# gylien/scale-letkf

Measured on AMD Instinct MI355X. Metric: grid-point LETKF solves/sec, higher is better.
Workload: dtype f64

## Files before the change

### __graft_entry__.py

```python
import importlib.util
import os
import subprocess
import sys

ROOT = os.path.dirname(os.path.abspath(__file__))
PKG_DIR = os.path.join(ROOT, "scale-letkf_amd")


def load_package():
    if "scale_letkf_amd" in sys.modules:
        return sys.modules["scale_letkf_amd"]
    spec = importlib.util.spec_from_file_location("scale_letkf_amd", os.path.join(PKG_DIR, "__init__.py"),
                                                  submodule_search_locations=[PKG_DIR])
    mod = importlib.util.module_from_spec(spec)
    sys.modules["scale_letkf_amd"] = mod
    spec.loader.exec_module(mod)
    return mod


def build():
    pkg = load_package()
    pkg.build()
    subprocess.check_call(["make", "-j4", "-C", PKG_DIR, "CHECKED=1"], stdout=2)
    subprocess.check_call(["make", "-C", os.path.join(ROOT, "oracle"), "oracle"])
    if os.path.isdir("/root/reference/common") and os.path.exists("/opt/rocm/bin/amdflang"):
        subprocess.check_call(["make", "-C", os.path.join(ROOT, "oracle"), "ref"])
    shim_mk = os.path.join(PKG_DIR, "fortran", "Makefile")
    if os.path.exists(shim_mk) and os.path.exists("/opt/rocm/bin/amdflang"):
        subprocess.check_call(["make", "-C", os.path.join(PKG_DIR, "fortran")])
    pkg.lib()


def smoke():
    import numpy as np
    import torch
    sys.path.insert(0, os.path.join(ROOT, "tests"))
    import _oracle
    from _cases import das_case, relerr
    pkg = load_package()
    assert torch.cuda.is_available(), "smoke() needs a GPU"
    dev = torch.device("cuda:0")
    c = das_case(k=20, nv=11, npts=16, nobs_tot=300, n_mean=40, seed=11)
    prm = _oracle.DasParams(k=20, nv=11, det_run=0, infl_adaptive=0, relax_to_inflated_prior=0, relax_alpha=0.0,
                            relax_alpha_spread=0.95, q_update_top=0.0, q_sprd_max=0.0, iv_p=4, iv_q_first=5,
                            iv_q_last=10, nthreads=1)
    ref = _oracle.das_points(prm, c["obs_off"], c["obs_idx"], c["rdiag"], c["rloc"], c["ensval"], c["dep"],
                             c["beta"], c["infl"], c["gues"], c["sp"], c["sm"], c["sv"])
    t = lambda a: torch.from_numpy(np.ascontiguousarray(a)).to(dev)
    ctx = pkg.Context(0, torch.cuda.current_stream().cuda_stream)
    anal = torch.zeros(c["gues"].size, dtype=torch.float64, device=dev)
    status = torch.full((c["npts"],), -1, dtype=torch.int32, device=dev)
    ctx.das_points(20, 11, t(c["obs_off"]), t(c["obs_idx"]), t(c["rdiag"]), t(c["rloc"]), t(c["ensval"]), c["kld"],
                   t(c["dep"]), t(c["infl"]), t(c["gues"]), anal, c["sp"], c["sm"], c["sv"], beta=t(c["beta"]),
                   relax_alpha_spread=0.95, status=status)
    torch.cuda.synchronize()
    assert int(status.abs().max()) == 0, status
    got = anal.cpu().numpy().reshape(11, c["nens"], c["npts"])[:, :20, :]
    exp = ref["anal"].reshape(11, c["nens"], c["npts"])[:, :20, :]
    err = relerr(got, exp)
    assert err < 1e-10, err
    print(f"smoke ok: 16 points, k=20, max rel err vs oracle {err:.2e}")


if __name__ == "__main__":
    build()
    print("build ok")
```

### scale-letkf_amd/csrc/letkf_jacobi_dev.h

```cpp
#pragma once
#include <hip/hip_runtime.h>

#include "letkf_lane_dev.h"

namespace letkf {
namespace jacobi_dev {

using namespace lane_dev;

typedef double v4d __attribute__((ext_vector_type(4)));

template <int NW>
__device__ __forceinline__ void psync() {
  if constexpr (NW == 1) wave_lds_sync();
  else __syncthreads();
}
template <int NW>
__device__ __forceinline__ bool pany(bool v) {
  if constexpr (NW == 1) return __builtin_amdgcn_ballot_w64(v) != 0ull;
  else return __syncthreads_or(v) != 0;
}

constexpr double kRotTol2W = 1e-30;
#ifndef LETKF_EARLY_TOL2
#define LETKF_EARLY_TOL2 1e-16
#endif
#ifndef LETKF_EARLY_T2
#define LETKF_EARLY_T2 1e-12
#endif
#ifndef LETKF_STOP_TOL2
#define LETKF_STOP_TOL2 1e-24
#endif
constexpr double kStopTol2W = LETKF_STOP_TOL2;
constexpr double kEarlyTol2W = LETKF_EARLY_TOL2;
constexpr double kEarlyT2W = LETKF_EARLY_T2;
constexpr double kEarlyTW = 1e-6;
static_assert(LETKF_EARLY_T2 == 1e-12, "kEarlyTW is its square root");

__device__ __forceinline__ double fast_rsqrt(double x) {
  const double y = __builtin_amdgcn_rsq(x);
  const double e = fma(-x * y, y, 1.0);
  const double q = e * fma(0.375, e, 0.5);
  return fma(y, q, y);
}
__device__ __forceinline__ double fast_rsqrt1(double x) { return __builtin_amdgcn_rsq(x); }
__device__ __forceinline__ double fast_rcp1(double x) { return __builtin_amdgcn_rcp(x); }
__device__ __forceinline__ double fast_rcp(double x) {
  double r = __builtin_amdgcn_rcp(x);
  double e = fma(-x, r, 1.0);
  r = fma(r, e, r);
  e = fma(-x, r, 1.0);
  return fma(r, e, r);
}

template <int CTRL>
__device__ __forceinline__ double dpp_shift_keep(double old, double v) {
  const int lo = __builtin_amdgcn_update_dpp(__double2loint(old), __double2loint(v), CTRL, 0xF, 0xF, false);
  const int hi = __builtin_amdgcn_update_dpp(__double2hiint(old), __double2hiint(v), CTRL, 0xF, 0xF, false);
  return __hiloint2double(hi, lo);
}
__device__ __forceinline__ double copy64(double v) {
  double t;
  asm("v_mov_b64 %0, %1" : "=v"(t) : "v"(v));
  return t;
}
__device__ __forceinline__ double slot_sum(double v) {
  const auto lo = __builtin_amdgcn_permlane32_swap(__double2loint(v), __double2loint(v), false, false);
  const auto hi = __builtin_amdgcn_permlane32_swap(__double2hiint(v), __double2hiint(v), false, false);
  return __hiloint2double(hi[0], lo[0]) + __hiloint2double(hi[1], lo[1]);
}

__device__ __forceinline__ double slot_sum_c64(double v) {
  const double t = copy64(v);
  const auto lo = __builtin_amdgcn_permlane32_swap(__double2loint(v), __double2loint(t), false, false);
  const auto hi = __builtin_amdgcn_permlane32_swap(__double2hiint(v), __double2hiint(t), false, false);
  return __hiloint2double(hi[0], lo[0]) + __hiloint2double(hi[1], lo[1]);
}

template <int NW>
__device__ __forceinline__ double slot_sum_nw(double v, double* xs, int& ph) {
  if constexpr (NW == 1) {
    return slot_sum_c64(v);
  } else {
    const int t = threadIdx.x & 127;
    xs[ph * 128 + t] = v;
    __syncthreads();
    const double o = xs[ph * 128 + (t ^ 64)];
    ph ^= 1;
    return v + o;
  }
}

template <int KR, int NW, int RC = 24, bool EARLY = true, bool INPLACE = false>
__device__ __forceinline__ int jacobi_split(double (&g)[KR], const int k, const int max_sweep, double* lds,
                                            int* pairs_out = nullptr, int* conv_out = nullptr, const double stop_tol2 = kStopTol2W) {
  static_assert(KR % 2 == 0, "row halves");
  constexpr int H = KR / 2;
  static_assert(RC % 2 == 0, "RC rows per conversion chunk: RC * 64 NW doubles of LDS");
  constexpr bool ENDS = NW == 1;
  static_assert(!ENDS || KR <= 64, "one wave: k <= 62, lane 31 stays switched off");
  constexpr int NL = 64 * NW;
  int lane = threadIdx.x & (NL - 1);
  if constexpr (NW == 2) asm volatile("" : "+v"(lane));
  const int slot = (NW == 1) ? (lane & 31) : (lane & 63), par = (NW == 1) ? (lane >> 5) : (lane >> 6);
  int ph = 0;
  const int ncol = (k + 1) & ~1;
  const int S = ncol >> 1;
  double xa[H], xb[H], xf[INPLACE ? 1 : H];
#pragma unroll
  for (int r0 = 0; r0 < KR; r0 += RC) {
    psync<NW>();
#pragma unroll
    for (int r = r0; r < r0 + RC && r < KR; ++r) lds[(r - r0) * NL + lane] = g[r];
    psync<NW>();
#pragma unroll
    for (int rr = r0 / 2; rr < (r0 + RC) / 2 && rr < H; ++rr) {
      const double2 v2 = *reinterpret_cast<const double2*>(&lds[(2 * rr + par - r0) * NL + 2 * slot]);
      xa[rr] = v2.x;
      xb[rr] = v2.y;
    }
  }
  int sweep = 0, pairs_done = 0, conv = 0;
  const bool act = slot < S;
  const bool rows = NW == 1 || act;
  if (NW == 2 || act) {
    const bool hasL = act && slot > 0, hasR = act && slot + 1 < S;
    const unsigned long long hasRm = __builtin_amdgcn_ballot_w64(hasR);
    double alA = 0.0, alB = 0.0, isA = 1.0, isB = 1.0, scA = 1.0, scB = 1.0;
    const double endR = hasR ? -0.0 : 1.0, endL = hasL ? -0.0 : 1.0;
    int quiet = 0, quiet2 = 0, pairs = 0, vph = 0;
    bool done = false;
    for (; sweep < max_sweep && !done; ++sweep) {
      double a0 = 0.0, b0 = 0.0;
      if (rows) {
#pragma unroll
        for (int rr = 0; rr < H; ++rr) {
          xa[rr] *= isA;
          xb[rr] *= isB;
          a0 = fma(xa[rr], xa[rr], a0);
          b0 = fma(xb[rr], xb[rr], b0);
        }
      }
      alA = slot_sum_nw<NW>(a0, lds, ph);
      alB = slot_sum_nw<NW>(b0, lds, ph);
      isA = isB = scA = scB = 1.0;
      for (int t = 0; t < ncol && !done; t += 2) {
        unsigned long long notconv = 0, notconv2 = 0;
        {
          double p0 = 0.0, p1 = 0.0;
          if (rows) {
#pragma unroll
            for (int rr = 0; rr < H; ++rr) {
              if (rr & 1) p1 = fma(xa[rr], xb[rr], p1);
              else p0 = fma(xa[rr], xb[rr], p0);
            }
          }
// ... 178 lines not shown
```

### scale-letkf_amd/csrc/letkf_trio.hip

```cpp
#include <hip/hip_runtime.h>
#include <stdint.h>

#include <type_traits>

#include "letkf_device.h"
#include "letkf_jacobi_dev.h"
#include "letkf_lane_dev.h"
#include "letkf_sched_dev.h"

namespace letkf {

namespace {

using namespace jacobi_dev;
using namespace lane_dev;

template <int KR, int P>
struct TrioLds {
  static constexpr int PSZ = (KR + 2) * KR;
  static constexpr int kSC = P > 3 ? 192 : 256;
  static constexpr int park = 0;
  static constexpr int lam = park + P * PSZ;
  static constexpr int st = lam + P * 32;
  static constexpr int work = st + P * 8;
// ... 42 lines not shown
    quiet[p] = quiet2[p] = pdone[p] = 0;
    sdone[p] = segm[p] == 0ull;
  }
  int pairs = 0;
  if (act) {
    const int colA = 2 * sin, colB = colA + 1;
    double xa[H], xb[H], xf[H];
#pragma unroll
    for (int rr = 0; rr < H; ++rr) {
      xa[rr] = base[colA * KR + 2 * rr + par];
      xb[rr] = base[colB * KR + 2 * rr + par];
    }
    const bool hasL = sin > 0, hasR = sin + 1 < S;
    const unsigned long long hasRm = __builtin_amdgcn_ballot_w64(hasR);
    double alA = 0.0, alB = 0.0, isA = 1.0, isB = 1.0, scA = 1.0, scB = 1.0;
    bool live = true;
    bool alldone = false;
    for (int sweep = 0; sweep < max_sweep && !alldone; ++sweep) {
      double a0 = 0.0, b0 = 0.0;
#pragma unroll
      for (int rr = 0; rr < H; ++rr) {
        xa[rr] *= isA;
        xb[rr] *= isB;
        a0 = fma(xa[rr], xa[rr], a0);
        b0 = fma(xb[rr], xb[rr], b0);
      }
      alA = slot_sum(a0);
      alB = slot_sum(b0);
      isA = isB = scA = scB = 1.0;
      for (int t = 0; t < ncol && !alldone; t += 2) {
        unsigned long long notconv = 0, notconv2 = 0;
        {
          double p0 = 0.0, p1 = 0.0;
#pragma unroll
          for (int rr = 0; rr < H; ++rr) {
            if (rr & 1) p1 = fma(xa[rr], xb[rr], p1);
            else p0 = fma(xa[rr], xb[rr], p0);
          }
          const double ga = slot_sum(p0 + p1) * (isA * isB);
          const double a = alA, b = alB;
          const double g2 = ga * ga, ab = a * b;
          notconv |= __builtin_amdgcn_ballot_w64(g2 > kStopTol2W * ab);
          const bool rot = live && g2 > kRotTol2W * ab;
          const double h = 0.5 * (b - a);
          const double x = fma(h, h, g2);
          const double den = fma(x, fast_rsqrt1(x), fabs(h));
          double tt = ga * fast_rcp1(copysign(den, h));
          tt = rot ? tt : 0.0;
          notconv2 |= __builtin_amdgcn_ballot_w64(g2 > kEarlyTol2W * ab) | __builtin_amdgcn_ballot_w64(fabs(tt) > kEarlyTW);
          const double w = fma(tt, tt, 1.0);
          const double c = fast_rsqrt(w);
          const double tg = tt * ga, wc = w * c;
          const double cA = tt * (isA * scB), cB = -tt * (isB * scA);
          const double nisA = isB * c, nscA = scB * wc, nisB = isA * c, nscB = scA * wc;
          alA = b + tg;
          alB = a - tg;
          isA = nisA;
          scA = nscA;
          isB = nisB;
          scB = nscB;
#pragma unroll
          for (int rr = 0; rr < H; ++rr) {
            asm("v_fma_f64 %0, %1, %2, %3" : "=&v"(xf[rr]) : "v"(cA), "v"(xa[rr]), "v"(xb[rr]));
            xa[rr] = fma(cB, xb[rr], xa[rr]);
          }
        }
        {
          double p0 = 0.0, p1 = 0.0;
#pragma unroll
          for (int rr = 0; rr < H; ++rr) xb[rr] = dpp_mov0<0x130>(xf[rr]);
          if (wrap) {
            if (lane == 31) {
#pragma unroll
              for (int rr = 0; rr < H; ++rr) xb[rr] = 0.0;
            }
          }
#pragma unroll
          for (int rr = 0; rr < H; ++rr) {
            if (rr & 1) p1 = fma(xa[rr], xb[rr], p1);
            else p0 = fma(xa[rr], xb[rr], p0);
          }
          const double alAr = dpp_mov0<0x130>(alA), isAr = dpp_mov0<0x130>(isA), scAr = dpp_mov0<0x130>(scA);
          const double ga = slot_sum(p0 + p1) * (isB * isAr);
          const double a = alB, b = alAr;
          const double g2 = ga * ga, ab = a * b;
          notconv |= __builtin_amdgcn_ballot_w64(g2 > kStopTol2W * ab) & hasRm;
          const bool rot = live && hasR && g2 > kRotTol2W * ab;
          const double h = 0.5 * (b - a);
          const double x = fma(h, h, g2);
          const double den = fma(x, fast_rsqrt1(x), fabs(h));
          double tt = ga * fast_rcp1(copysign(den, h));
          tt = rot ? tt : 0.0;
          notconv2 |= (__builtin_amdgcn_ballot_w64(g2 > kEarlyTol2W * ab) | __builtin_amdgcn_ballot_w64(fabs(tt) > kEarlyTW)) & hasRm;
          const double w = fma(tt, tt, 1.0);
          const double c = fast_rsqrt(w);
          const double tg = tt * ga, wc = w * c;
          const double q1 = dpp_mov0<0x138>(-tt * scB), q2 = dpp_mov0<0x138>(isB * c),
                       q3 = dpp_mov0<0x138>(scB * wc), q4 = dpp_mov0<0x138>(a - tg);
          const double coefR = hasR ? tt * (isB * scAr) : 1.0;
          const double coefL = hasL ? q1 * isA : 1.0;
          if (hasR) {
            alB = b + tg;
            isB = isAr * c;
            scB = scAr * wc;
          }
          if (hasL) {
            alA = q4;
            isA = q2;
            scA = q3;
          }
#pragma unroll
          for (int rr = 0; rr < H; ++rr) {
            xb[rr] = fma(coefR, xa[rr], xb[rr]);
            xa[rr] = dpp_mov0<0x138>(xa[rr]);
          }
          if (wrap) {
            if (lane == 32) {
#pragma unroll
              for (int rr = 0; rr < H; ++rr) xa[rr] = 0.0;
            }
          }
#pragma unroll
          for (int rr = 0; rr < H; ++rr) xa[rr] = fma(coefL, xf[rr], xa[rr]);
        }
        ++pairs;
        alldone = true;
#pragma unroll
        for (int p = 0; p < P; ++p) {
          if (!sdone[p]) {
            quiet[p] = (notconv & segm[p]) ? 0 : quiet[p] + 1;
            quiet2[p] = (notconv2 & segm[p]) ? 0 : quiet2[p] + 1;
            if (quiet[p] >= S || quiet2[p] >= S) {
              sdone[p] = true;
              pdone[p] = pairs;
              if (seg == p) live = false;
            }
          }
          alldone = alldone && sdone[p];
        }
      }
    }
    double sa = 0.0, sb = 0.0;
#pragma unroll
    for (int rr = 0; rr < H; ++rr) {
      xa[rr] *= isA;
      xb[rr] *= isB;
      sa = fma(xa[rr], xa[rr], sa);
      sb = fma(xb[rr], xb[rr], sb);
    }
    sa = slot_sum(sa);
    sb = slot_sum(sb);
    const double lamA = sqrt(sa), lamB = sqrt(sb);
    const double ilA = sa > 0.0 ? 1.0 / lamA : 0.0, ilB = sb > 0.0 ? 1.0 / lamB : 0.0;
#pragma unroll
    for (int rr = 0; rr < H; ++rr) {
      base[colA * KR + 2 * rr + par] = xa[rr] * ilA;
      base[colB * KR + 2 * rr + par] = xb[rr] * ilB;
    }
    if (par == 0) {
      double* lv = slice + L::lam + seg * 32;
      lv[colA] = lamA;
      lv[colB] = lamB;
    }
    if (sin == 0 && par == 0) {
      int mypd = 0;
#pragma unroll
      for (int p = 0; p < P; ++p)
        if (seg == p) mypd = sdone[p] ? pdone[p] : 0;
      const int pr = mypd > 0 ? mypd : pairs;
      slice[L::st + seg * 8 + ST_SWEEPS] = (double)((pr + S - 1) / S);
      slice[L::st + seg * 8 + ST_CONV] = mypd > 0 ? 1.0 : 0.0;
    }
  }
  wave_lds_sync();
}

struct TrioHead {
  long pt;
  long o0, o1;
  double beta;
};
struct TrioList {
  int iob[4];
  double rlv[4], rdv[4];
};
__device__ __forceinline__ TrioHead trio_head(const PointArgs& A, const long pt) {
  TrioHead h;
  h.pt = pt;
  h.o0 = h.o1 = 0;
  h.beta = 1.0;
  if (pt >= 0) {
    h.o0 = A.obs_off[pt];
    h.o1 = A.obs_off[pt + 1];
    if (A.beta) h.beta = A.beta[pt];
  }
  return h;
}
template <int kSC>
__device__ __forceinline__ TrioList trio_list(const PointArgs& A, const TrioHead& h) {
  TrioList l;
  const int lane = threadIdx.x & 63;
  const int n = (int)(h.o1 - h.o0);
  const int ns = (h.pt >= 0 && h.beta != 0.0) ? (n < kSC ? n : kSC) : 0;
#pragma unroll
  for (int ps = 0; ps < 4; ++ps) {
    const int i = ps * 64 + lane;
    l.iob[ps] = 0;
    l.rdv[ps] = 1.0;
    l.rlv[ps] = 0.0;
    if (i < ns) {
      const long e = h.o0 + i;
      l.iob[ps] = A.obs_idx[e];
      l.rlv[ps] = A.rloc_l[e];
      l.rdv[ps] = A.rdiag_l[e];
    }
  }
  return l;
}

template <int KR, int P>
__device__ __forceinline__ int trio_front(const PointArgs& A, const TrioHead& hd, const TrioList& pl, const int sub, double* slice, const int k, const bool warm, TrioProf& pf) {
  using L = TrioLds<KR, P>;
  constexpr int RS = KR - 16;
  constexpr int NBLK = RS > 0 ? 2 : 1;
  constexpr int RSA = RS > 0 ? RS : 1;
  const int lane = threadIdx.x & 63;
  const double km1 = (double)(k - 1);
  const long pt = hd.pt;
  const long o0 = hd.o0;
  const int n = __builtin_amdgcn_readfirstlane((int)(hd.o1 - hd.o0));
  const double beta = uniform(hd.beta);
  if (beta == 0.0) return 0;
  if (n == 0) return 1;
  const double* g0 = A.gues + pt * A.sp;
  bool qskip = false;
  if (A.q_update_top > 0.0) qskip = g0[k * A.sm + A.iv_p * A.sv] < A.q_update_top;
  int v0 = 0;
  while (v0 < A.nv && (!((A.var_mask >> v0) & 1u) || (qskip && v0 >= A.iv_q_first && v0 <= A.iv_q_last))) ++v0;
  const double infl_old = (v0 < A.nv) ? A.infl[pt + A.infl_sv * (long)v0] : 1.0;

  v4d acc = v4d{0.0, 0.0, 0.0, 0.0};
  [[maybe_unused]] double accS[RSA][NBLK];
  double accD[NBLK], accDD[NBLK], accP = 0.0, p3 = 0.0;
#pragma unroll
  for (int I = 0; I < NBLK; ++I) {
    accD[I] = accDD[I] = 0.0;
#pragma unroll
    for (int a = 0; a < RSA; ++a) accS[a][I] = 0.0;
  }
  int q = lane >> 4, c16 = lane & 15;
  asm volatile("" : "+v"(q), "+v"(c16));
  constexpr int kSC = L::kSC;
  double* stg = slice + L::work;
  bool rowok[NBLK];
  long mo[NBLK];
#pragma unroll
  for (int I = 0; I < NBLK; ++I) {
    const int m = 16 * I + c16;
    rowok[I] = m < k;
    mo[I] = rowok[I] ? m : 0;
  }
  struct Step {
    double f[NBLK];
    double sw, dsw, ddsw;
  };
  const double* ybase = A.ensval;
  auto run_steps = [&](const int nsp) {
    const int nch = nsp >> 2;
    auto fetch = [&](const int c, Step& t) {
      const bool ok = c < nch;
      const int i = 4 * (ok ? c : 0) + q;
      const double2 a2 = *reinterpret_cast<const double2*>(&stg[4 * i]);
      const double2 b2 = *reinterpret_cast<const double2*>(&stg[4 * i + 2]);
      const long rb = __double_as_longlong(a2.x);
      t.sw = ok ? a2.y : 0.0;
      t.dsw = ok ? b2.x : 0.0;
      t.ddsw = ok ? b2.y : 0.0;
#pragma unroll
      for (int I = 0; I < NBLK; ++I) t.f[I] = ybase[rb + mo[I]];
    };
    auto mma = [&](const Step& t) {
      double y[NBLK];
#pragma unroll
      for (int I = 0; I < NBLK; ++I) {
        double v = t.f[I] * t.sw;
        if (I > 0 || k < 16) v = rowok[I] ? v : 0.0;
        y[I] = v;
        accD[I] = fma(v, t.dsw, accD[I]);
        accDD[I] = fma(v, t.ddsw, accDD[I]);
      }
      accP = fma(t.dsw, t.dsw, accP);
      acc = __builtin_amdgcn_mfma_f64_16x16x4f64(y[0], y[0], acc, 0, 0, 0);
      if constexpr (RS > 0) {
        auto strip_row = [&](auto a_) {
          constexpr int a = decltype(a_)::value;
          if constexpr (a < RS) {
#pragma unroll
            for (int I = 0; I < NBLK; ++I) {
              if (a == 0 && I == 0) fmac_row_bcast<a, true>(accS[a][I], y[NBLK - 1], y[I]);
              else fmac_row_bcast<a, false>(accS[a][I], y[NBLK - 1], y[I]);
            }
          }
        };
        strip_row(std::integral_constant<int, 0>{});
        strip_row(std::integral_constant<int, 1>{});
        strip_row(std::integral_constant<int, 2>{});
        strip_row(std::integral_constant<int, 3>{});
      }
    };
#ifndef TRIO_GRAM_DEPTH
#define TRIO_GRAM_DEPTH 5
#endif
    constexpr int PD = TRIO_GRAM_DEPTH;
    Step ts[PD];
#pragma unroll
// ... 527 lines not shown
```

### scale-letkf_amd/csrc/letkf_wave_dev.h

```cpp
#pragma once
#include <hip/hip_runtime.h>
#include <stdint.h>

#include <type_traits>

#include "letkf_device.h"
#include "letkf_search_dev.h"
#include "letkf_jacobi_dev.h"
#include "letkf_lane_dev.h"
#include "letkf_sched_dev.h"

namespace letkf {

using namespace jacobi_dev;
using namespace lane_dev;

template <int NW, int OP>
__device__ __forceinline__ double preduce(double v, double* red, int& slot) {
  v = (OP == 0) ? wave_sum(v) : (OP == 1) ? wave_max(v) : wave_min(v);
  if constexpr (NW == 1) {
    return v;
  } else {
    if ((threadIdx.x & 63) == 0) red[2 * slot + (threadIdx.x >> 6)] = v;
    __syncthreads();
// ... 226 lines not shown
      const double2 v2 = *reinterpret_cast<const double2*>(&mine[r]);
      g[r] = wlane < KR ? v2.x : 0.0;
      g[r + 1] = wlane < KR ? v2.y : 0.0;
    }
  }
  wave_lds_sync();
}

#ifndef LETKF_WARM_STRIP
#define LETKF_WARM_STRIP 1
#endif
template <int KR>
__device__ __forceinline__ void warm_start_product_strip(double (&g)[KR], const double* __restrict__ qslot, double* cb) {
  constexpr int NBF = KR / 16;
  constexpr int RS = KR - 16 * NBF;
  static_assert(KR % 2 == 0 && KR <= 50 && RS == 2 && NBF == 3, "A must fit the LDS slice; the narrow block is a pair (16-byte reads); the pin below");
  constexpr int KS = (KR + 3) / 4;
  constexpr int PD = (KS < 6) ? KS : 6;
  const int wlane = threadIdx.x & 63;
  const int q = wlane >> 4, c = wlane & 15;
  struct QOp {
    double b[NBF];
    double2 be;
  };
  struct AOp {
    double a[NBF];
    double2 ae;
  };
  unsigned long long qaddr = reinterpret_cast<unsigned long long>(qslot + q * 64 + c);
  asm volatile("" : "+v"(qaddr));
  const gdouble* qp = (const gdouble*)qaddr;
  auto ldq = [&](const int s) {
    QOp t;
#pragma unroll
    for (int J = 0; J < NBF; ++J) t.b[J] = 0.0;
    t.be = double2{0.0, 0.0};
    if (4 * s + 3 < KR || 4 * s + q < KR) {
      const gdouble* a = qp + (size_t)s * 256;
#pragma unroll
      for (int J = 0; J < NBF; ++J) t.b[J] = a[16 * J];
      const v2d_t e2 = *(const gdouble2*)(a + (16 * NBF - c));
      t.be = double2{e2.x, e2.y};
    }
    return t;
  };
  auto lda = [&](const int s) {
    AOp t;
#pragma unroll
    for (int I = 0; I < NBF; ++I) t.a[I] = 0.0;
    t.ae = double2{0.0, 0.0};
    if (4 * s + 3 < KR || 4 * s + q < KR) {
      const double* a = cb + (4 * s + q) * KR;
#pragma unroll
      for (int I = 0; I < NBF; ++I) t.a[I] = a[16 * I + c];
      t.ae = *reinterpret_cast<const double2*>(a + 16 * NBF);
    }
    return t;
  };
  QOp qr[PD];
#pragma unroll
  for (int s = 0; s < PD; ++s) qr[s] = ldq(s);
  wave_lds_sync();
  if (wlane < KR) {
    double* mine = cb + wlane * KR;
#pragma unroll
    for (int r = 0; r < KR; r += 2) *reinterpret_cast<double2*>(&mine[r]) = double2{g[r], g[r + 1]};
  }
  wave_lds_sync();
  v4d acc[NBF * NBF];
#pragma unroll
  for (int t = 0; t < NBF * NBF; ++t) acc[t] = v4d{0.0, 0.0, 0.0, 0.0};
  double rs[RS][NBF], cs[RS][NBF], cn[RS][RS];
#pragma unroll
  for (int e = 0; e < RS; ++e) {
#pragma unroll
    for (int I = 0; I < NBF; ++I) rs[e][I] = cs[e][I] = 0.0;
#pragma unroll
    for (int f = 0; f < RS; ++f) cn[e][f] = 0.0;
  }
  AOp ar[2];
  ar[0] = lda(0);
#pragma unroll
  for (int s = 0; s < KS; ++s) {
    if (s + 1 < KS) ar[(s + 1) & 1] = lda(s + 1);
    const AOp a4 = ar[s & 1];
    const QOp b4 = qr[s % PD];
    const double ae[RS] = {a4.ae.x, a4.ae.y}, be[RS] = {b4.be.x, b4.be.y};
#pragma unroll
    for (int I = 0; I < NBF; ++I)
#pragma unroll
      for (int J = 0; J < NBF; ++J) acc[NBF * I + J] = __builtin_amdgcn_mfma_f64_16x16x4f64(a4.a[I], b4.b[J], acc[NBF * I + J], 0, 0, 0);
#pragma unroll
    for (int e = 0; e < RS; ++e) {
#pragma unroll
      for (int I = 0; I < NBF; ++I) {
        rs[e][I] = fma(ae[e], b4.b[I], rs[e][I]);
        cs[e][I] = fma(a4.a[I], be[e], cs[e][I]);
      }
#pragma unroll
      for (int f = 0; f < RS; ++f) cn[e][f] = fma(ae[e], be[f], cn[e][f]);
    }
    if (s + PD < KS) qr[s % PD] = ldq(s + PD);
    asm volatile(""
                 : "+v"(rs[0][0]), "+v"(rs[0][1]), "+v"(rs[0][2]), "+v"(rs[1][0]), "+v"(rs[1][1]), "+v"(rs[1][2]), "+v"(cs[0][0]),
                   "+v"(cs[0][1]), "+v"(cs[0][2]), "+v"(cs[1][0]), "+v"(cs[1][1]), "+v"(cs[1][2]), "+v"(cn[0][0]), "+v"(cn[0][1]),
                   "+v"(cn[1][0]), "+v"(cn[1][1])::"memory");
  }
  auto fold = [](double v) {
    v += __shfl_xor(v, 16);
    v += __shfl_xor(v, 32);
    return v;
  };
#pragma unroll
  for (int e = 0; e < RS; ++e) {
#pragma unroll
    for (int I = 0; I < NBF; ++I) {
      rs[e][I] = fold(rs[e][I]);
      cs[e][I] = fold(cs[e][I]);
    }
#pragma unroll
    for (int f = 0; f < RS; ++f) cn[e][f] = fold(cn[e][f]);
  }
  wave_lds_sync();
#pragma unroll
  for (int J = 0; J < NBF; ++J) {
    double* col = cb + (16 * J + c) * KR;
#pragma unroll
    for (int I = 0; I < NBF; ++I)
#pragma unroll
      for (int reg = 0; reg < 4; ++reg) col[16 * I + 4 * reg + q] = acc[NBF * I + J][reg];
    if (q == 0) *reinterpret_cast<double2*>(&col[16 * NBF]) = double2{rs[0][J], rs[1][J]};
  }
  if (q == 1) {
#pragma unroll
    for (int e = 0; e < RS; ++e)
#pragma unroll
      for (int I = 0; I < NBF; ++I) cb[(16 * NBF + e) * KR + 16 * I + c] = cs[e][I];
  }
  if (wlane == 32) {
#pragma unroll
    for (int f = 0; f < RS; ++f) *reinterpret_cast<double2*>(&cb[(16 * NBF + f) * KR + 16 * NBF]) = double2{cn[0][f], cn[1][f]};
  }
  wave_lds_sync();
  {
    const double* mine = cb + (wlane < KR ? wlane : 0) * KR;
#pragma unroll
    for (int r = 0; r < KR; r += 2) {
      const double2 v2 = *reinterpret_cast<const double2*>(&mine[r]);
      g[r] = wlane < KR ? v2.x : 0.0;
      g[r + 1] = wlane < KR ? v2.y : 0.0;
    }
  }
  wave_lds_sync();
}

__host__ __device__ constexpr int wave_kmin(int KR, int NW) {
  return NW == 1 ? (KR == 16 ? 1 : KR == 20 ? 17 : KR == 32 ? 17 : KR == 48 ? 33 : KR == 50 ? 49 : KR == 64 ? 51 : 1)
                 : (KR == 64 ? 63 : KR == 80 ? 65 : KR == 100 ? 81 : 1);
}

__host__ __device__ constexpr bool wave_small(int KR, int NW) { return NW == 1 && KR <= 20; }
__host__ __device__ constexpr int wave_base_doubles(int KR, int NW) { return wave_small(KR, NW) ? 1280 : 1536 * NW; }
__host__ __device__ constexpr int wave_jacobi_rc(int KR, int NW) { return wave_small(KR, NW) ? KR : 24; }
__host__ __device__ constexpr int wave_ob_rows(int KR) { return KR <= 20 ? 32 : 64; }
#ifndef LETKF_SMALL_OCC
#define LETKF_SMALL_OCC 2
#endif
__host__ __device__ constexpr int wave_occupancy(int KR, int NW) { return NW == 1 ? (wave_small(KR, NW) ? LETKF_SMALL_OCC : 2) : 1; }

__host__ __device__ inline int wave_slice_doubles(int KR, int nv, int NW) {
  const int nb = nv + 2;
  int tile = kTnW * 64;
  const int vb = KR * kVld;
  if (vb > tile) tile = vb;
  int bmat = ((nb + 1) & ~1) * KR;
  if (kChunk * KR > bmat) bmat = kChunk * KR;
  const int cb = kChunk * ((nb + 1) & ~1);
  const int small = 3 * kTnW + 8 * nv + 16;
  if (tile + bmat < wave_base_doubles(KR, NW)) bmat = wave_base_doubles(KR, NW) - tile;
  int tot = tile + bmat + cb + small + 8;
  if (NW == 1 && KR <= 50 && tot < (KR - 1) * KR + 64) tot = (KR - 1) * KR + 64;
  if (NW == 1 && KR < 32 && tot < 32 * KR + 64 * ((KR + 3) / 4) + 128 + 16 * wave_ob_rows(KR)) tot = 32 * KR + 64 * ((KR + 3) / 4) + 128 + 16 * wave_ob_rows(KR);
  if (NW == 1 && KR <= 50 && tot < 32 * KR + 64 * ((KR + 3) / 4) + 128)
    tot = 32 * KR + 64 * ((KR + 3) / 4) + 128;
  return (tot + 1) & ~1;
}

#ifdef LETKF_WAVE_PROF
#define PROF_DECL unsigned long long prof_t[10] = {0, 0, 0, 0, 0, 0, 0, 0, 0, 0}; unsigned long long prof_last = __builtin_amdgcn_s_memtime(); const unsigned long long prof_t0 = prof_last; int prof_units = 0;
#define PROF_MARK(i) { const unsigned long long t_ = __builtin_amdgcn_s_memtime(); prof_t[i] += t_ - prof_last; prof_last = t_; }
#define PROF_FLUSH if (A.prof && wlane == 0) { for (int i_ = 0; i_ < 10; ++i_) atomicAdd(&A.prof[i_], prof_t[i_]); \
    atomicMax(&A.prof[10], ~prof_t0); atomicMax(&A.prof[11], (unsigned long long)__builtin_amdgcn_s_memtime()); \
    atomicAdd(&A.prof[12 + (prof_units < 11 ? prof_units : 11)], 1ull); atomicAdd(&A.prof[24], (unsigned long long)prof_units); }
#define PROF_UNIT ++prof_units;
#else
#define PROF_DECL
#define PROF_MARK(i)
#define PROF_FLUSH
#define PROF_UNIT
#endif

#ifdef LETKF_CHECKED
#define LETKF_CHECK(ok, code, val, lim) letkf_check_fail(A.prof, (ok), (code), (long)(val), (long)(lim))
__device__ __forceinline__ bool letkf_check_fail(unsigned long long* rec, const bool ok, const int code, const long val, const long lim) {
  if (!ok && rec && atomicCAS(&rec[0], 0ull, (unsigned long long)code) == 0ull) {
    rec[1] = blockIdx.x;
    rec[2] = (unsigned long long)val;
    rec[3] = (unsigned long long)lim;
  }
  return ok;
}
#else
#define LETKF_CHECK(ok, code, val, lim) true
#endif

template <int KR, int NV, bool KKOUT, int NW, int FUSED>
__global__ void __launch_bounds__(NW == 1 ? 256 : 128, wave_occupancy(KR, NW)) letkf_wave_kernel(const PointArgs A) {
  extern __shared__ __attribute__((aligned(16))) double smem[];
  constexpr int NB = NV + 2;
  constexpr int NBP = (NB + 1) & ~1;
  constexpr int NL = 64 * NW;
  int lane = threadIdx.x & (NL - 1);
  int wlane = threadIdx.x & 63;
  const int wvp = (NW == 1) ? 0 : (threadIdx.x >> 6);
  const int wv = (NW == 1) ? (threadIdx.x >> 6) : 0;
  const int k = A.k;
  const int nv = A.nv;
  const double km1 = (double)(k - 1);

  double* slice = smem + (size_t)wv * wave_slice_doubles(KR, NV, NW);
  int tile_sz = kTnW * 64;
  if (KR * kVld > tile_sz) tile_sz = KR * kVld;
  int bmat_sz = NBP * KR;
  if (kChunk * KR > bmat_sz) bmat_sz = kChunk * KR;
  if (tile_sz + bmat_sz < wave_base_doubles(KR, NW)) bmat_sz = wave_base_doubles(KR, NW) - tile_sz;
  double* vbuf = slice;
  double* bmat = slice + tile_sz;
  double* cbuf = bmat + bmat_sz;
  double* wrow = cbuf + kChunk * NBP;
  double* xsm = wrow + 3 * kTnW;
  double* xmean = xsm;
  double* xdet = xsm + NV;
  double* red = xsm + 8 * NV + 16;
  int rslot = 0;

  constexpr int PPW = (NW == 1) ? 4 : 1;
  const int run_len = A.run_len;
  const long S = A.warm_stride, nA = A.npts / S;
  double* uws = (run_len > 1) ? A.warm_ws + ((size_t)blockIdx.x * PPW + wv) * ((size_t)KR * NL) + lane : nullptr;
  PROF_DECL
#ifdef LETKF_WAVE_PROF
  long Bstat = blockIdx.x;
#endif
  bool first_draw = true;
  int pend = 0;
  long next_rid = 0;
  for (;;) {
   long rid;
   int ir0 = 0, ir1 = run_len;
#ifdef LETKF_WAVE_PROF
   if (!A.sched) {
     const long nruns = S * ((nA + run_len - 1) / run_len);
     const long nB = (nruns + PPW - 1) / PPW;
     if (Bstat >= nB) break;
     rid = xcd_remap(Bstat, nB) * PPW + wv;
     Bstat += gridDim.x;
     if (rid >= nruns) continue;
   } else
#endif
   if (pend > 0) {
     rid = next_rid++;
     --pend;
   } else {
     int code;
     const int slot0 = first_draw ? (int)(blockIdx.x >> 3) * PPW + wv : -1;
     if constexpr (NW == 1) {
       code = sched_next(A.plan, A.sched, (int)(blockIdx.x & 7), slot0);
     } else {
       int* slot_ = reinterpret_cast<int*>(red + 6);
       __syncthreads();
       if (threadIdx.x < 64) {
         const int g = sched_next(A.plan, A.sched, (int)(blockIdx.x & 7), slot0);
         if (threadIdx.x == 0) *slot_ = g;
       }
       __syncthreads();
       code = *slot_;
     }
     first_draw = false;
     PROF_MARK(9)
     if (code < 0) break;
     PROF_UNIT
     if (code & 4) {
       ir0 = (code & 3) * run_len >> 2;
       ir1 = ((code & 3) + 1) * run_len >> 2;
     }
     rid = (long)(code >> 3) * A.plan.ub;
     const long left = A.plan.nruns - rid;
     pend = (int)(left < A.plan.ub ? left : A.plan.ub) - 1;
     next_rid = rid + 1;
   }
   const long rchunk = rid / S, rb = rid - rchunk * S;
   const long ra0 = rchunk * run_len;
   bool have_u = false;
   [[maybe_unused]] int pre_n = -1;
   for (int ir = ir0; ir < ir1; ++ir) {
    if (ra0 + ir >= nA) break;
// ... 518 lines not shown
      }
#pragma unroll
      for (int I = 0; I < NBLK; ++I) {
        psync<NW>();
#pragma unroll
        for (int pass = 0; pass < NW; ++pass) {
          if (pass == 1) __syncthreads();
          if (wvp == pass) {
            if constexpr (STRIP) {
              {
                if (I < NBLK - 1) {
#pragma unroll
                  for (int a = 0; a < 16; ++a) abuf[(16 * (NBLK - 1) + a) * LDA + c16] = a < RS ? accS[a][I] : 0.0;
                } else {
#pragma unroll
                  for (int J = 0; J < NBLK; ++J)
#pragma unroll
                    for (int a = 0; a < RS; ++a) abuf[(16 * J + c16) * LDA + a] = accS[a][J];
                }
              }
            }
#pragma unroll
            for (int J = 0; J < NBF; ++J) {
              if (STRIP && I == NBLK - 1) continue;
              const int ti = I <= J ? I : J, tj = I <= J ? J : I;
              const int t = ti * NBF - ti * (ti - 1) / 2 + (tj - ti);
#pragma unroll
              for (int reg = 0; reg < 4; ++reg) {
                const int a = q + 4 * reg, b = c16;
                double* dst = (I <= J) ? &abuf[(16 * J + b) * LDA + a] : &abuf[(16 * J + a) * LDA + b];
                if (pass == 0) *dst = acc[t][reg];
                else *dst += acc[t][reg];
              }
            }
          }
        }
        psync<NW>();
        if constexpr (NW == 1) {
          const int lrow = lane < 16 * NBLK ? lane : 16 * NBLK - 1;
          const bool mine = lane < 16 * NBLK;
#pragma unroll
          for (int e = 0; e < 16; e += 2) {
            if (16 * I + e < KR) {
              const double2 v2 = *reinterpret_cast<const double2*>(&abuf[lrow * LDA + e]);
              g[16 * I + e] = v2.x;
              g[16 * I + e + 1] = v2.y;
            }
          }
          if constexpr (!STRIP) {
            if ((k >> 4) == I) {
              const double t = abuf[lrow * LDA + (k & 15)];
              racc = mine ? t : racc;
            }
            if (((k + 1) >> 4) == I) {
              const double t = abuf[lrow * LDA + ((k + 1) & 15)];
              rdacc = mine ? t : rdacc;
            }
          }
        } else if (lane < 16 * NBLK) {
#pragma unroll
          for (int e = 0; e < 16; e += 2) {
            if (16 * I + e < KR) {
              const double2 v2 = *reinterpret_cast<const double2*>(&abuf[lane * LDA + e]);
              g[16 * I + e] = v2.x;
              g[16 * I + e + 1] = v2.y;
            }
          }
          if constexpr (!STRIP) {
            if ((k >> 4) == I) racc = abuf[lane * LDA + (k & 15)];
            if (((k + 1) >> 4) == I) rdacc = abuf[lane * LDA + ((k + 1) & 15)];
          }
        }
        if constexpr (!STRIP) {
          if ((k >> 4) == I) p1 = abuf[k * LDA + (k & 15)];
        }
      }
      psync<NW>();
#pragma unroll
      for (int r = 0; r < KR; ++r)
        if (r >= k || lane >= k || lane >= 16 * NBLK) g[r] = 0.0;
      const double shift = km1 / infl_old;
      double diag = 0.0;
#pragma unroll
      for (int r = 0; r < KR; ++r) {
        if (r == lane && lane < k) {
          diag = g[r];
          g[r] += shift;
        }
      }
      double parm1 = 0.0, parm2 = 0.0, parm3 = 0.0;
      if (A.infl_adaptive) {
        parm1 = p1;
        parm3 = preduce<NW, 0>(p3, red, rslot);
        parm2 = preduce<NW, 0>(lane < k ? diag : 0.0, red, rslot) / km1;
      }

      PROF_MARK(2)
      if (have_u && !(A.warm_dbg & 1)) {
        if constexpr (LETKF_WARM_STRIP && NW == 1 && KR == 50) warm_start_product_strip<KR>(g, uws - lane, slice);
        else if constexpr (NW == 1 && KR <= 50) warm_start_product_mfma<KR>(g, uws - lane, slice);
        else warm_start_product<KR, NW>(g, uws, k, slice);
      }
      PROF_MARK(3)
      sweeps = jacobi_split<KR, NW, wave_jacobi_rc(KR, NW), true, LETKF_INPLACE_NW(KR, NW)>(g, k, A.max_sweep, slice, nullptr, &jconv);
      asm volatile("" : "+v"(racc), "+v"(rdacc), "+v"(moff));
      PROF_MARK(4)

      double ss = 0.0;
#pragma unroll
      for (int r = 0; r < KR; ++r) ss = fma(g[r], g[r], ss);
      lam = sqrt(ss);
      colvalid = ss > 0.0;
      const double il = colvalid ? 1.0 / lam : 0.0;
#pragma unroll
      for (int r = 0; r < KR; ++r) g[r] *= il;

      if (A.infl_adaptive) {
        const double parm4 = (parm1 - parm3) / parm2 - infl_old;
        const double tq = (infl_old * parm2 + parm3) / parm2;
        const double sigma_o = 2.0 / parm3 * (tq * tq);
        const double gain = 0.04 * 0.04 / (sigma_o + 0.04 * 0.04);
        p1 = infl_old + gain * parm4;
      }
      }
    }
    constexpr bool MAPPLY = !KKOUT && NW == 1 && KR <= 50 && NV > 0 && NB <= 14;
    constexpr int kBmRows = 4 * ((KR + 3) / 4), kBmOff = 32 * KR;
    constexpr int kObOff = (32 * KR >= 1024) ? 0 : kBmOff + 16 * kBmRows + 128;
    if constexpr (!MAPPLY) {
      if (!solved) {
#pragma unroll
        for (int r = 0; r < KR; ++r) g[r] = (r == lane && lane < k) ? 1.0 : 0.0;
      }
    }
    const double infl_new = (A.infl_adaptive && n > 0) ? p1 : infl_old;
    double xv[NV > 0 ? NV : 1];
    double xm_l = 0.0, xd_l = 0.0;
    if constexpr (MAPPLY) {
      const double* gp = g0 + moff;
#pragma unroll
      for (int v = 0; v < NV; ++v) {
        xv[v] = (lane < k) ? *gp : 0.0;
        gp += A.sv;
      }
      if (lane < NV) {
        xm_l = g0[k * A.sm + lane * A.sv];
        xd_l = A.det_run ? g0[(k + 1) * A.sm + lane * A.sv] : 0.0;
      }
      asm volatile("" ::: "memory");
    }
    {
      if (uws && solved && !(A.warm_dbg & 2)) {
        unsigned long long pa = reinterpret_cast<unsigned long long>(uws);
#pragma unroll
        for (int r = 0; r < KR; ++r) {
          if ((r & 7) == 0) asm volatile("" : "+v"(pa));
          ((gdouble*)pa)[(size_t)(r & 7) * NL] = g[r];
          if ((r & 7) == 7) pa += 8 * NL * sizeof(double);
        }
      }
    }

    int st = 0;
    {
      const double lmx = preduce<NW, 1>(colvalid ? lam : 0.0, red, rslot);
      const double lmn = preduce<NW, 2>(colvalid ? lam : 1e300, red, rslot);
      if (!jconv && A.max_sweep >= 60) st = 1;
      else if (!(lmx > 0.0)) st = 2;
      else if (lmn < lmx * 1.4901161193847656e-08) st = 3;
    }
    have_u = uws != nullptr && st == 0 && solved;
    const double sc1 = colvalid ? sqrt(km1 / lam) : 0.0;
    const double sc2 = colvalid ? 1.0 / lam : 0.0;

    PROF_MARK(5)
    const int mrow_l = lane < KR ? lane : KR - 1;
    double cf[NV > 0 ? NV : 1];
    double out[NB];
    if constexpr (MAPPLY) {
      if (!solved) {
        out[0] = 0.0;
        out[1] = 0.0;
        wave_lds_sync();
        if (lane < kBmRows) {
#pragma unroll
          for (int v = 0; v < NV; ++v) slice[kBmOff + lane * 16 + 2 + v] = xv[v];
        }
        wave_lds_sync();
#pragma unroll
        for (int v = 0; v < NV; ++v) {
          out[2 + v] = sc1 * xv[v];
          double cfv = 1.0;
          if (A.relax_alpha != 0.0) {
            cfv = 1.0 - A.relax_alpha;
          } else if (A.relax_alpha_spread != 0.0) {
            const double parm = A.relax_to_inflated_prior ? A.infl[pt + A.infl_sv * (long)v] : 1.0;
            const double var_g = wave_sum(xv[v] * xv[v]);
            const double var_a = var_g * uniform(sc2);
            if (var_g > 0.0 && var_a > 0.0)
              cfv = A.relax_alpha_spread * sqrt(var_g * parm / (var_a * km1)) - A.relax_alpha_spread + 1.0;
          }
          cf[v] = uniform(cfv);
          if (A.rtps_out && lane == 0 && ((A.var_mask >> v) & 1u)) {
            const bool skipv = qskip && v >= A.iv_q_first && v <= A.iv_q_last;
            A.rtps_out[pt + A.infl_sv * (long)v] = (A.relax_alpha == 0.0 && A.relax_alpha_spread != 0.0 && !skipv) ? cfv : 1.0;
          }
        }
      } else {
      constexpr int KS = (KR + 3) / 4;
      constexpr int BR = 4 * KS;
      double* vh = slice;
      double* bm = slice + 32 * KR;
      double* scl = bm + BR * 16;
      int q = wlane >> 4, c = wlane & 15;
      asm volatile("" : "+v"(q), "+v"(c));
      wave_lds_sync();
      {
        if (lane < BR) {
          double brow[16];
          brow[0] = (lane < k) ? racc : 0.0;
          brow[1] = (lane < k) ? rdacc : 0.0;
#pragma unroll
          for (int b = 2; b < 16; ++b) brow[b] = (b - 2 < NV) ? xv[b - 2 < NV ? b - 2 : 0] : 0.0;
          double* row = bm + lane * 16;
#pragma unroll
          for (int b = 0; b < 16; b += 2) *reinterpret_cast<double2*>(&row[b]) = double2{brow[b], brow[b + 1]};
        }
        *reinterpret_cast<double2*>(&scl[2 * lane]) = double2{sc2, sc1};
      }
      v4d accO[4];
#pragma unroll
      for (int t = 0; t < 4; ++t) accO[t] = v4d{0.0, 0.0, 0.0, 0.0};
      double va = 0.0, vg = 0.0;
#pragma unroll
      for (int h = 0; h < 2; ++h) {
        if (32 * h < KR) {
          wave_lds_sync();
          if ((lane >> 5) == h && lane < KR) {
            double* mine = vh + (lane - 32 * h) * KR;
#pragma unroll
            for (int r = 0; r < KR; r += 2) *reinterpret_cast<double2*>(&mine[r]) = double2{g[r], g[r + 1]};
          }
          wave_lds_sync();
          v4d accU[2];
          accU[0] = v4d{0.0, 0.0, 0.0, 0.0};
          accU[1] = v4d{0.0, 0.0, 0.0, 0.0};
#pragma unroll
          for (int s_ = 0; s_ < KS; ++s_) {
            const double bq = bm[(4 * s_ + q) * 16 + c];
            if (h == 0) vg = fma(bq, bq, vg);
#pragma unroll
            for (int il = 0; il < 2; ++il) {
              if (32 * h + 16 * il < KR) {
                const double a = vh[(16 * il + c) * KR + 4 * s_ + q];
                accU[il] = __builtin_amdgcn_mfma_f64_16x16x4f64(a, bq, accU[il], 0, 0, 0);
              }
            }
          }
#pragma unroll
          for (int il = 0; il < 2; ++il) {
#pragma unroll
            for (int reg = 0; reg < 4; ++reg) {
              const int s_ = 4 * (2 * h + il) + reg;
              if (4 * s_ < KR) {
                const int j = 4 * s_ + q;
                const double2 sc = *reinterpret_cast<const double2*>(&scl[2 * j]);
                const double u = accU[il][reg];
                va = fma(u * u, sc.x, va);
                const double cv = u * (c < 2 ? sc.x : sc.y);
                const double* a = vh + (j - 32 * h) * KR + 4 * c;
                const double2 lo = *reinterpret_cast<const double2*>(a);
                const double2 hi = *reinterpret_cast<const double2*>(a + 2);
                accO[0] = __builtin_amdgcn_mfma_f64_16x16x4f64(lo.x, cv, accO[0], 0, 0, 0);
                accO[1] = __builtin_amdgcn_mfma_f64_16x16x4f64(lo.y, cv, accO[1], 0, 0, 0);
                accO[2] = __builtin_amdgcn_mfma_f64_16x16x4f64(hi.x, cv, accO[2], 0, 0, 0);
                accO[3] = __builtin_amdgcn_mfma_f64_16x16x4f64(hi.y, cv, accO[3], 0, 0, 0);
              }
            }
          }
        }
      }
      PROF_MARK(6)
      va += wshfl_xor(va, 16);
      va += wshfl_xor(va, 32);
      vg += wshfl_xor(vg, 16);
      vg += wshfl_xor(vg, 32);
      {
        const int v = c - 2;
        const bool isv = c >= 2 && c < NB;
        double cfv = 1.0;
        if (A.relax_alpha != 0.0) {
          cfv = 1.0 - A.relax_alpha;
        } else if (A.relax_alpha_spread != 0.0) {
          const double parm = (A.relax_to_inflated_prior && isv) ? A.infl[pt + A.infl_sv * (long)v] : 1.0;
          if (vg > 0.0 && va > 0.0) cfv = A.relax_alpha_spread * sqrt(vg * parm / (va * km1)) - A.relax_alpha_spread + 1.0;
        }
        if (A.rtps_out && q == 0 && isv && ((A.var_mask >> v) & 1u)) {
          const bool skipv = qskip && v >= A.iv_q_first && v <= A.iv_q_last;
          A.rtps_out[pt + A.infl_sv * (long)v] = (A.relax_alpha == 0.0 && A.relax_alpha_spread != 0.0 && !skipv) ? cfv : 1.0;
        }
#pragma unroll
        for (int vv = 0; vv < NV; ++vv) cf[vv] = readlane_d(cfv, 2 + vv);
      }
      wave_lds_sync();
      double* ob = slice + kObOff;
      constexpr int OBR = wave_ob_rows(KR);
// ... 233 lines not shown
```

Measured before the change: 9.454 million.

## Sort saved warm-start eigenvectors by eigenvalue before storing them

When eigenvectors are saved for warm-starting the next Jacobi solve, they are now permuted into descending eigenvalue order. Each column's rank comes from a cross-lane comparison of a key built from the eigenvalue's high bits with a lane-index tiebreak. The trio path and the single-wave path both write columns at their ranked position. The aim is a warm start whose column order matches the next point's spectrum, so Jacobi needs fewer sweeps, at the cost of extra shuffles or readlanes per solve. The build script also gains a PROF=1 make step.

```diff
diff --git a/__graft_entry__.py b/__graft_entry__.py
--- a/__graft_entry__.py
+++ b/__graft_entry__.py
@@ -22,6 +22,7 @@
     pkg = load_package()
     pkg.build()
     subprocess.check_call(["make", "-j4", "-C", PKG_DIR, "CHECKED=1"], stdout=2)
+    subprocess.check_call(["make", "-j4", "-C", PKG_DIR, "PROF=1"], stdout=2)
     subprocess.check_call(["make", "-C", os.path.join(ROOT, "oracle"), "oracle"])
     if os.path.isdir("/root/reference/common") and os.path.exists("/opt/rocm/bin/amdflang"):
         subprocess.check_call(["make", "-C", os.path.join(ROOT, "oracle"), "ref"])
diff --git a/scale-letkf_amd/csrc/letkf_jacobi_dev.h b/scale-letkf_amd/csrc/letkf_jacobi_dev.h
--- a/scale-letkf_amd/csrc/letkf_jacobi_dev.h
+++ b/scale-letkf_amd/csrc/letkf_jacobi_dev.h
@@ -2,6 +2,10 @@
 #include <hip/hip_runtime.h>
 
 #include "letkf_lane_dev.h"
+
+#ifndef LETKF_WARM_SORT
+#define LETKF_WARM_SORT 1
+#endif
 
 namespace letkf {
 namespace jacobi_dev {
diff --git a/scale-letkf_amd/csrc/letkf_trio.hip b/scale-letkf_amd/csrc/letkf_trio.hip
--- a/scale-letkf_amd/csrc/letkf_trio.hip
+++ b/scale-letkf_amd/csrc/letkf_trio.hip
@@ -218,15 +218,33 @@
     sb = slot_sum(sb);
     const double lamA = sqrt(sa), lamB = sqrt(sb);
     const double ilA = sa > 0.0 ? 1.0 / lamA : 0.0, ilB = sb > 0.0 ? 1.0 / lamB : 0.0;
+    int dstA = colA, dstB = colB;
+#if LETKF_WARM_SORT
+    {
+      const unsigned keyA = (sa > 0.0 ? ((unsigned)__double2hiint(lamA) & ~63u) : 0u) | (unsigned)(63 - colA);
+      const unsigned keyB = (sb > 0.0 ? ((unsigned)__double2hiint(lamB) & ~63u) : 0u) | (unsigned)(63 - colB);
+      const int seg0 = slot - sin;
+      dstA = dstB = 0;
+#pragma unroll
+      for (int i = 0; i < H; ++i) {
+        const int src = seg0 + (i < S ? i : 0);
+        const unsigned oa = (unsigned)__shfl((int)keyA, src, 64), ob = (unsigned)__shfl((int)keyB, src, 64);
+        if (i < S) {
+          dstA += (oa > keyA ? 1 : 0) + (ob > keyA ? 1 : 0);
+          dstB += (oa > keyB ? 1 : 0) + (ob > keyB ? 1 : 0);
+        }
+      }
+    }
+#endif
 #pragma unroll
     for (int rr = 0; rr < H; ++rr) {
-      base[colA * KR + 2 * rr + par] = xa[rr] * ilA;
-      base[colB * KR + 2 * rr + par] = xb[rr] * ilB;
+      base[dstA * KR + 2 * rr + par] = xa[rr] * ilA;
+      base[dstB * KR + 2 * rr + par] = xb[rr] * ilB;
     }
     if (par == 0) {
       double* lv = slice + L::lam + seg * 32;
-      lv[colA] = lamA;
-      lv[colB] = lamB;
+      lv[dstA] = lamA;
+      lv[dstB] = lamB;
     }
     if (sin == 0 && par == 0) {
       int mypd = 0;
diff --git a/scale-letkf_amd/csrc/letkf_wave_dev.h b/scale-letkf_amd/csrc/letkf_wave_dev.h
--- a/scale-letkf_amd/csrc/letkf_wave_dev.h
+++ b/scale-letkf_amd/csrc/letkf_wave_dev.h
@@ -402,6 +402,20 @@
     }
   }
   wave_lds_sync();
+}
+
+template <int KR>
+__device__ __forceinline__ int warm_rank(const double lam, const bool colvalid, const int lane) {
+  constexpr int NLN = KR < 64 ? KR : 64;
+  const unsigned tie = 63u - (unsigned)(lane & 63);
+  unsigned key = colvalid ? (((unsigned)__double2hiint(lam) & ~63u) | tie) : tie;
+  int rank = 0;
+#pragma unroll
+  for (int i = 0; i < NLN; ++i) {
+    if ((i & 7) == 0) asm volatile("" : "+v"(key), "+v"(rank));
+    rank += ((unsigned)__builtin_amdgcn_readlane((int)key, i) > key) ? 1 : 0;
+  }
+  return lane < NLN ? rank : lane;
 }
 
 __host__ __device__ constexpr int wave_kmin(int KR, int NW) {
@@ -1226,6 +1240,10 @@
     {
       if (uws && solved && !(A.warm_dbg & 2)) {
         unsigned long long pa = reinterpret_cast<unsigned long long>(uws);
+        if constexpr (LETKF_WARM_SORT && NW == 1) {
+          const int rk = warm_rank<KR>(lam, colvalid, lane);
+          pa += (long long)(((A.warm_dbg & 16) ? lane : rk) - lane) * (long long)sizeof(double);
+        }
 #pragma unroll
         for (int r = 0; r < KR; ++r) {
           if ((r & 7) == 0) asm volatile("" : "+v"(pa));
```

Result: faster. 9.815 million, median of 6 (+3.8%).
